# michaelnny/muzero

Measured on AMD Instinct MI355X. Metric: self-play MCTS sims/sec (env-steps/sec = value / sims_per_move), higher is better.
Workload: dtype f32

## Files before the change

muzero_amd/csrc/mz_search_fast.h:

```cpp
#pragma once
#include <type_traits>

#include "mz_search.h"

namespace mz {

#ifndef MZ_FAST_RD
#define MZ_FAST_RD 3
#endif
#ifndef MZ_FAST_RD256
#define MZ_FAST_RD256 4
#endif
#ifndef MZ_FAST_RD_GEN
#define MZ_FAST_RD_GEN 2
#endif
constexpr int fast_rd(int planes, int ac) { return planes == 256 ? MZ_FAST_RD256 : (ac == 2 ? MZ_FAST_RD : MZ_FAST_RD_GEN); }
#ifndef MZ_FAST_HW
#define MZ_FAST_HW 1
#endif
constexpr bool kFastHW = MZ_FAST_HW != 0;
#ifndef MZ_FAST_SC
#define MZ_FAST_SC 1
#endif
#ifndef MZ_FAST_AX
#define MZ_FAST_AX 1
#endif
constexpr bool kFastSC = MZ_FAST_SC != 0, kFastAX = MZ_FAST_AX != 0;

struct FastWeights {
    const float4* stream;
    unsigned bytes;
    const float* wact;
};

typedef unsigned int u32x4 __attribute__((ext_vector_type(4)));

struct WSrc {
    __amdgpu_buffer_rsrc_t r;
    int base;
    int cur;
};

__device__ __forceinline__ WSrc make_wsrc(const void* p, unsigned bytes, int base) {
    WSrc w;
    w.r = __builtin_amdgcn_make_buffer_rsrc(const_cast<void*>(p), 0, (int)bytes, 0x00020000);
    w.base = base;
    w.cur = base;
    return w;
}

__device__ __forceinline__ float4 bload(const WSrc& w, int voff, int block) {
    const u32x4 v = __builtin_amdgcn_raw_buffer_load_b128(w.r, voff, w.base + block * 1024, 0);
    return make_float4(__uint_as_float(v.x), __uint_as_float(v.y), __uint_as_float(v.z), __uint_as_float(v.w));
}

__device__ __forceinline__ float comp(const float4& v, int i) { return i == 0 ? v.x : (i == 1 ? v.y : (i == 2 ? v.z : v.w)); }

template <int P, int TR, int TV, int RD, int XG_ = 5>
struct FastCfg {
    static constexpr int NT = P / 64;
    static constexpr int XG = XG_;
    static constexpr int I_D1 = 0, I_D2 = I_D1 + XG, I_R1 = I_D2 + 4, I_R2 = I_R1 + 4, I_V1 = I_R2 + TR, I_V2 = I_V1 + 4, I_END = I_V2 + TV;
    static constexpr int SL = (I_END + RD - 1) / RD * RD;
};

template <typename C, int RD, int I>
__device__ __forceinline__ void prefetch_slot(float4 (&ring)[RD][C::NT], WSrc& ws, int voff) {
    constexpr int T = (I + RD - 1) % C::SL;
#ifdef MZ_EXP_NOLOAD
    return;
#endif
    if constexpr (T < C::I_END) {
        int so = ws.cur;
        asm volatile("" : "+s"(so));
        ws.cur = so + (T + 1 == C::I_END ? -(C::I_END - 1) : 1) * C::NT * 1024;
#pragma unroll
        for (int j = 0; j < C::NT; j++) {
            const u32x4 v = __builtin_amdgcn_raw_buffer_load_b128(ws.r, voff + (j & 3) * 1024, so + (j >> 2) * 4096, 0);
            ring[T % RD][j] = make_float4(__uint_as_float(v.x), __uint_as_float(v.y), __uint_as_float(v.z), __uint_as_float(v.w));
        }
    }
}

template <int NT, bool LDS_READ, int NV = 0>
__device__ __forceinline__ void slot_schedule() {
    if (LDS_READ) __builtin_amdgcn_sched_group_barrier(0x100, 1, 0);
#pragma unroll
    for (int i = 0; i < NT; i++) {
        __builtin_amdgcn_sched_group_barrier(0x020, 1, 0);
        if (NV == 0) {
            __builtin_amdgcn_sched_group_barrier(0x008, 4, 0);
        } else {
#pragma unroll
            for (int m = 0; m < 2; m++) {
                __builtin_amdgcn_sched_group_barrier(0x008, 2, 0);
                __builtin_amdgcn_sched_group_barrier(0x002, NV, 0);
            }
        }
    }
    if (NV == 0) __builtin_amdgcn_sched_barrier(0);
    else __builtin_amdgcn_sched_barrier(0);
}

struct NoHook {
    template <int K>
    __device__ __forceinline__ void stage() {}
};

template <typename C, int RD, int I0, int G, int KG, bool FROM_LDS, int NV = 0, typename Hook = NoHook, int HK0 = 0>
struct WideSlots {
    static __device__ __forceinline__ void run(float4 (&ring)[RD][C::NT], WSrc& ws, int voff, const float4 (&xs)[5], const f32x4 (&hin)[4],
                                               int last_steps, f32x4 (&acc)[C::NT], Hook& hook) {
        constexpr int NT = C::NT, I = I0 + G;
        prefetch_slot<C, RD, I>(ring, ws, voff);
        hook.template stage<HK0 + G>();
        float b[4];
        if (FROM_LDS) {
            const float4 x = xs[G];
            b[0] = x.x; b[1] = x.y; b[2] = x.z; b[3] = x.w;
        } else {
            b[0] = hin[G][0]; b[1] = hin[G][1]; b[2] = hin[G][2]; b[3] = hin[G][3];
        }
        const float4(&w)[NT] = ring[I % RD];
#pragma unroll
        for (int j = 0; j < NT; j++) acc[j] = __builtin_amdgcn_mfma_f32_16x16x4f32(w[j].x, b[0], acc[j], 0, 0, 0);
        if (G + 1 < KG || last_steps > 1) {
#pragma unroll
            for (int j = 0; j < NT; j++) acc[j] = __builtin_amdgcn_mfma_f32_16x16x4f32(w[j].y, b[1], acc[j], 0, 0, 0);
        }
        if (G + 1 < KG || last_steps > 2) {
#pragma unroll
            for (int j = 0; j < NT; j++) acc[j] = __builtin_amdgcn_mfma_f32_16x16x4f32(w[j].z, b[2], acc[j], 0, 0, 0);
        }
        if (G + 1 < KG || last_steps > 3) {
#pragma unroll
            for (int j = 0; j < NT; j++) acc[j] = __builtin_amdgcn_mfma_f32_16x16x4f32(w[j].w, b[3], acc[j], 0, 0, 0);
        }
        slot_schedule<NT, false, NV>();
        if constexpr (G + 1 < KG) WideSlots<C, RD, I0, G + 1, KG, FROM_LDS, NV, Hook, HK0>::run(ring, ws, voff, xs, hin, last_steps, acc, hook);
    }
};

template <typename C, int RD, int I0, int D, int TO, int NV = 0, typename Hook = NoHook, int HK0 = 0>
struct SplitSlots {
    static __device__ __forceinline__ void run(float4 (&ring)[RD][C::NT], WSrc& ws, int voff, const f32x4 (&hin)[C::NT], f32x4 (&acc)[TO],
                                               Hook& hook) {
        constexpr int NT = C::NT, I = I0 + D, KPS = NT / TO;
        static_assert(NT % TO == 0, "tiles per slot");
        prefetch_slot<C, RD, I>(ring, ws, voff);
        hook.template stage<HK0 + D>();
        const float4(&w)[NT] = ring[I % RD];
#pragma unroll
        for (int kk = 0; kk < KPS; kk++) {
            const int kb = D * KPS + kk;
#pragma unroll
            for (int st = 0; st < 4; st++) {
#pragma unroll
                for (int t = 0; t < TO; t++)
                    acc[t] = __builtin_amdgcn_mfma_f32_16x16x4f32(comp(w[kk * TO + t], st), hin[kb][st], acc[t], 0, 0, 0);
            }
        }
        slot_schedule<NT, false, NV>();
        if constexpr (D + 1 < TO) SplitSlots<C, RD, I0, D + 1, TO, NV, Hook, HK0>::run(ring, ws, voff, hin, acc, hook);
    }
};

template <typename C, int RD, int I>
struct PadSlots {
    static __device__ __forceinline__ void run(float4 (&ring)[RD][C::NT], WSrc& ws, int voff) {
        if constexpr (I < C::SL) {
            prefetch_slot<C, RD, I>(ring, ws, voff);
            __builtin_amdgcn_sched_barrier(0);
            PadSlots<C, RD, I + 1>::run(ring, ws, voff);
        }
    }
};

__device__ __forceinline__ float opaque_f32(unsigned int bits) {
    asm("" : "+s"(bits));
    return __uint_as_float(bits);
}
__device__ __forceinline__ float fmin2(float a, float b) { return __builtin_amdgcn_fmed3f(a, b, opaque_f32(0xff800000u)); }
__device__ __forceinline__ float fmax2(float a, float b) { return __builtin_amdgcn_fmed3f(a, b, opaque_f32(0x7f800000u)); }
typedef unsigned int u32x2 __attribute__((ext_vector_type(2)));
__device__ __forceinline__ float rows_min(float v) {
    u32x2 r = __builtin_amdgcn_permlane16_swap(__float_as_uint(v), __float_as_uint(v), false, false);
    v = fmin2(__uint_as_float(r[0]), __uint_as_float(r[1]));
    r = __builtin_amdgcn_permlane32_swap(__float_as_uint(v), __float_as_uint(v), false, false);
    return fmin2(__uint_as_float(r[0]), __uint_as_float(r[1]));
}
__device__ __forceinline__ float rows_max(float v) {
    u32x2 r = __builtin_amdgcn_permlane16_swap(__float_as_uint(v), __float_as_uint(v), false, false);
    v = fmax2(__uint_as_float(r[0]), __uint_as_float(r[1]));
    r = __builtin_amdgcn_permlane32_swap(__float_as_uint(v), __float_as_uint(v), false, false);
    return fmax2(__uint_as_float(r[0]), __uint_as_float(r[1]));
}

template <int N>
__device__ __forceinline__ void relu_tiles(f32x4 (&a)[N]) {
    const float inf = opaque_f32(0x7f800000u);
#pragma unroll
    for (int j = 0; j < N; j++) {
#pragma unroll
        for (int r = 0; r < 4; r++) a[j][r] = __builtin_amdgcn_fmed3f(a[j][r], 0.0f, inf);
    }
}

template <int TO>
__device__ __forceinline__ float head_logit(const float* PB, int n, int e) {
    const int t = n >> 4, idx = ((t * 64 + ((n & 15) >> 2) * 16 + e) << 2) + (n & 3);
    const float c0 = PB[idx], c1 = PB[idx + TO * 256], c2 = PB[idx + 2 * TO * 256], c3 = PB[idx + 3 * TO * 256];
    return ((c0 + c1) + c2) + c3;
}

template <int NT>
__device__ __forceinline__ void root_inference_fast(const MlpNet& net, const MlpLds& o, float* lds, float4* scr, float* hid0, float* pi0, int tid, int wave,
                                                    int lane, bool active) {
    const int q = lane >> 4;
    const float* bias = lds;
    MZ_ROOT_TS_START();
    f32x4 h1[NT];
    if (active) {
        const MlpLayer& L0 = net.L[L_REP0];
        const float4* wp = reinterpret_cast<const float4*>(L0.w) + (size_t)(NT * wave) * L0.kg * 64 + lane;
#pragma unroll
        for (int j = 0; j < NT; j++) {
            const float4 bv = *reinterpret_cast<const float4*>(bias + L0.b_lds + (NT * wave + j) * 16 + q * 4);
            h1[j] = f32x4{bv.x, bv.y, bv.z, bv.w};
        }
        float4 w0[NT], w1[NT];
#pragma unroll
        for (int j = 0; j < NT; j++) w0[j] = ldg4(&wp[(size_t)j * L0.kg * 64]);
        for (int g = 0; g < L0.kg; g += 2) {
            const int g1 = g + 1 < L0.kg ? g + 1 : g, g2 = g + 2 < L0.kg ? g + 2 : g;
#pragma unroll
            for (int j = 0; j < NT; j++) w1[j] = ldg4(&wp[((size_t)j * L0.kg + g1) * 64]);
            mma_block<NT>(h1, w0, reinterpret_cast<const float4*>(lds + o.X)[g * 64 + lane], g + 1 < L0.kg ? 4 : L0.last_steps);
#pragma unroll
            for (int j = 0; j < NT; j++) w0[j] = ldg4(&wp[((size_t)j * L0.kg + g2) * 64]);
            if (g + 1 < L0.kg) mma_block<NT>(h1, w1, reinterpret_cast<const float4*>(lds + o.X)[(g + 1) * 64 + lane], g + 2 < L0.kg ? 4 : L0.last_steps);
        }
        relu_tiles<NT>(h1);
        MZ_ROOT_TS(0);
        const MlpLayer& L1 = net.L[L_REP1];
        const float4* wq = reinterpret_cast<const float4*>(L1.w) + lane;
        f32x4 acc2[4];
#pragma unroll
        for (int t = 0; t < 4; t++) {
            const float4 bv = *reinterpret_cast<const float4*>(bias + L1.b_lds + t * 16 + q * 4);
            acc2[t] = wave == 0 ? f32x4{bv.x, bv.y, bv.z, bv.w} : f32x4{0.0f, 0.0f, 0.0f, 0.0f};
        }
        float4 wa[4], wb[4];
#pragma unroll
        for (int t = 0; t < 4; t++) wa[t] = ldg4(&wq[((size_t)t * L1.kg + NT * wave) * 64]);
#pragma unroll
        for (int kk = 0; kk < NT; kk += 2) {
#pragma unroll
            for (int t = 0; t < 4; t++) wb[t] = ldg4(&wq[((size_t)t * L1.kg + NT * wave + (kk + 1 < NT ? kk + 1 : kk)) * 64]);
#pragma unroll
            for (int st = 0; st < 4; st++) {
#pragma unroll
                for (int t = 0; t < 4; t++) acc2[t] = __builtin_amdgcn_mfma_f32_16x16x4f32(comp(wa[t], st), h1[kk][st], acc2[t], 0, 0, 0);
            }
#pragma unroll
            for (int t = 0; t < 4; t++) wa[t] = ldg4(&wq[((size_t)t * L1.kg + NT * wave + (kk + 2 < NT ? kk + 2 : kk)) * 64]);
            if (kk + 1 < NT) {
#pragma unroll
                for (int st = 0; st < 4; st++) {
#pragma unroll
                    for (int t = 0; t < 4; t++) acc2[t] = __builtin_amdgcn_mfma_f32_16x16x4f32(comp(wb[t], st), h1[kk + 1][st], acc2[t], 0, 0, 0);
                }
            }
        }
#pragma unroll
        for (int t = 0; t < 4; t++) scr[(wave * 4 + t) * 64 + lane] = make_float4(acc2[t][0], acc2[t][1], acc2[t][2], acc2[t][3]);
    }
    __syncthreads();
    MZ_ROOT_TS(1);
    if (active) {
        auto tile = [&](int t) {
            const float4 c0 = scr[(0 * 4 + t) * 64 + lane], c1 = scr[(1 * 4 + t) * 64 + lane], c2 = scr[(2 * 4 + t) * 64 + lane], c3 = scr[(3 * 4 + t) * 64 + lane];
            return f32x4{((c0.x + c1.x) + c2.x) + c3.x, ((c0.y + c1.y) + c2.y) + c3.y, ((c0.z + c1.z) + c2.z) + c3.z, ((c0.w + c1.w) + c2.w) + c3.w};
        };
        const f32x4 h0 = tile(0), h1_ = tile(1), h2 = tile(2), h3 = tile(3);
        float mn = h0[0], mx = h0[0];
#pragma unroll
        for (int r = 0; r < 4; r++) { mn = fmin2(h0[r], mn); mx = fmax2(h0[r], mx); }
#pragma unroll
        for (int r = 0; r < 4; r++) { mn = fmin2(h1_[r], mn); mx = fmax2(h1_[r], mx); }
#pragma unroll
        for (int r = 0; r < 4; r++) { mn = fmin2(h2[r], mn); mx = fmax2(h2[r], mx); }
#pragma unroll
        for (int r = 0; r < 4; r++) { mn = fmin2(h3[r], mn); mx = fmax2(h3[r], mx); }
        mn = rows_min(mn);
        mx = rows_max(mx);
        const float d = (mx - mn) + 1e-8f;
        f32x4 hw = h0;
        if (wave == 1) hw = h1_;
        if (wave == 2) hw = h2;
        if (wave == 3) hw = h3;
        const float4 hs = make_float4((hw[0] - mn) / d, (hw[1] - mn) / d, (hw[2] - mn) / d, (hw[3] - mn) / d);
        reinterpret_cast<float4*>(lds + o.HS)[wave * 64 + lane] = hs;
        if (hid0) *reinterpret_cast<float4*>(hid0 + wave * 16 + q * 4) = hs;
    }
    __syncthreads();
    MZ_ROOT_TS(2);
    if (active) {
        const MlpLayer& L2 = net.L[L_POL0];
        const float4* wp = reinterpret_cast<const float4*>(L2.w) + (size_t)(NT * wave) * L2.kg * 64 + lane;
        f32x4 p1[NT];
#pragma unroll
        for (int j = 0; j < NT; j++) {
            const float4 bv = *reinterpret_cast<const float4*>(bias + L2.b_lds + (NT * wave + j) * 16 + q * 4);
            p1[j] = f32x4{bv.x, bv.y, bv.z, bv.w};
        }
        float4 w0[NT], w1[NT];
#pragma unroll
        for (int j = 0; j < NT; j++) w0[j] = ldg4(&wp[(size_t)j * L2.kg * 64]);
#pragma unroll
        for (int g = 0; g < 4; g += 2) {
#pragma unroll
            for (int j = 0; j < NT; j++) w1[j] = ldg4(&wp[((size_t)j * L2.kg + g + 1) * 64]);
            mma_block_full<NT>(p1, w0, reinterpret_cast<const float4*>(lds + o.HS)[g * 64 + lane]);
#pragma unroll
            for (int j = 0; j < NT; j++) w0[j] = ldg4(&wp[((size_t)j * L2.kg + (g + 2 < 4 ? g + 2 : g)) * 64]);
            mma_block_full<NT>(p1, w1, reinterpret_cast<const float4*>(lds + o.HS)[(g + 1) * 64 + lane]);
        }
        relu_tiles<NT>(p1);
        MZ_ROOT_TS(3);
        const MlpLayer& L3 = net.L[L_POL1];
        const float4* wq = reinterpret_cast<const float4*>(L3.w) + (size_t)(NT * wave) * 64 + lane;
        const float4 bv = *reinterpret_cast<const float4*>(bias + L3.b_lds + q * 4);
        f32x4 accp = wave == 0 ? f32x4{bv.x, bv.y, bv.z, bv.w} : f32x4{0.0f, 0.0f, 0.0f, 0.0f};
        float4 wv[NT];
#pragma unroll
        for (int kk = 0; kk < NT; kk++) wv[kk] = ldg4(&wq[kk * 64]);
#pragma unroll
        for (int kk = 0; kk < NT; kk++) {
#pragma unroll
            for (int st = 0; st < 4; st++) accp = __builtin_amdgcn_mfma_f32_16x16x4f32(comp(wv[kk], st), p1[kk][st], accp, 0, 0, 0);
        }
        scr[wave * 64 + lane] = make_float4(accp[0], accp[1], accp[2], accp[3]);
    }
    __syncthreads();
    MZ_ROOT_TS(4);
    if (active && wave == 0) {
        const float4 c0 = scr[lane], c1 = scr[64 + lane], c2 = scr[128 + lane], c3 = scr[192 + lane];
        float* pl = lds + o.LG + (lane & 15) * o.lg_stride + q * 4;
        pl[0] = ((c0.x + c1.x) + c2.x) + c3.x; pl[1] = ((c0.y + c1.y) + c2.y) + c3.y;
        pl[2] = ((c0.z + c1.z) + c2.z) + c3.z; pl[3] = ((c0.w + c1.w) + c2.w) + c3.w;
    }
    __syncthreads();
    if (active) row_softmax(lds + o.LG + (tid >> 4) * o.lg_stride, pi0 + (tid >> 4) * net.A, net.A, tid & 15);
    __syncthreads();
    MZ_ROOT_TS(5);
}

template <int P, int TR, int TV, bool FUSE = false, int AC = 0, bool HW = false, bool SPB = false>
__global__ __launch_bounds__(HW ? 2 * WG_THREADS : WG_THREADS) __attribute__((amdgpu_waves_per_eu(HW ? 2 : 1, HW ? 2 : 1))) void k_search_fast(const SearchParams Pm, const FastWeights FW) {
    constexpr bool TWO = AC == 2;
    constexpr int RD = fast_rd(P, AC);
    constexpr bool SC = AC == 10 && kFastSC, AX = AC == 10 && kFastAX;
    using C = FastCfg<P, SC ? 0 : TR, SC ? 0 : TV, RD, AX ? 4 : 5>;
    constexpr int NT = C::NT;
    extern __shared__ __attribute__((aligned(16))) unsigned char smem[];
    float* lds = reinterpret_cast<float*>(smem);
    const int wave8 = __builtin_amdgcn_readfirstlane((int)threadIdx.x >> 6);
    const bool main_w = !HW || wave8 < WG_WAVES;
    const int tid = threadIdx.x & (WG_THREADS - 1), e = tid >> 4, a0 = tid & 15, lane = tid & 63;
    const int wave = wave8 & (WG_WAVES - 1);
    const int env_g = blockIdx.x * TILE_E + e;
    const bool env_ok = env_g < Pm.B;
    if constexpr (FUSE) { if (main_w) fused_env_pre(Pm, a0, env_g, env_ok); }
    const bool hwx = HW && (Pm.hwx & 1) != 0;
    const bool hwx2 = HW && (Pm.hwx & 2) != 0;
    const MlpNet& net = Pm.net;
    const int root_layers[4] = {L_REP0, L_REP1, L_POL0, L_POL1};
    const float warm = main_w ? prefetch_root_weights(net, root_layers, 4, tid) : 0.0f;
    const MlpLds& o = Pm.o;
    float* pi0 = reinterpret_cast<float*>(smem + Pm.t_pi0);
    const float** src = reinterpret_cast<const float**>(smem + Pm.t_ptr);
    float** dst = reinterpret_cast<float**>(smem + Pm.t_ptr) + 16;

    MZ_STAMP_DECL
    MZ_STAMP_START();
    if (main_w) {
        stage_biases(net, lds, tid);
        if (!HW) tree2_init(smem, Pm, tid, env_ok, env_g);
        if (a0 == 0) {
            src[e] = env_ok ? Pm.obs + (size_t)env_g * net.in_dim : nullptr;
            dst[e] = env_ok ? Pm.hidden + (size_t)env_g * Pm.NN * net.H : nullptr;
        }
    }
    __syncthreads();
    MZ_STAMP(2);
    if (!HW) root_noise_lanes(smem, Pm, e, a0, env_g, env_ok);
    if (main_w) load_obs(net, lds + o.X, src, tid);
    __syncthreads();
    MZ_STAMP(15);
    if (HW && !main_w) {
        tree2_init(smem, Pm, tid, env_ok, env_g);
        root_noise_lanes(smem, Pm, e, a0, env_g, env_ok);
    }
    {
        const int e2r = lane & 15, env2r = blockIdx.x * TILE_E + e2r;
        float* hid0 = (main_w && env2r < Pm.B) ? Pm.hidden + (size_t)env2r * Pm.NN * 64 : nullptr;
        root_inference_fast<NT>(net, o, lds, reinterpret_cast<float4*>(lds + o.H1), hid0, pi0, tid, wave, lane, main_w);
    }
    if (Pm.S < 0) Pm.hidden[0] = warm;
    __syncthreads();
    {
        MZ_ROOT_TS_START();
        SearchParams Pr = Pm;
        if constexpr (AC == 10 || AC == 4) Pr.A = AC;
        if constexpr (TWO) Pr.A = 2;
        if constexpr (SPB) { Pr.noise_mode = 2; Pr.has_mask = 1; }
        if (main_w && env_ok) root_prior_group(smem, Pr, e, a0, env_g);
        MZ_ROOT_TS(6);
    }

    const int voff = lane * 16;
    WSrc ws = make_wsrc(FW.stream, FW.bytes, wave * C::SL * NT * 1024);
    ws.cur = ws.base + (RD - 1) * NT * 1024;
    float4 ring[RD][NT];
    if (main_w) {
#pragma unroll
        for (int i = 0; i < RD - 1; i++) {
#pragma unroll
            for (int j = 0; j < NT; j++) ring[i][j] = bload(ws, voff, i * NT + j);
        }
    }
    const int x_last = AX ? 4 : (TWO ? 1 : net.L[L_DYN0].last_steps);
    const int e2 = lane & 15, q = lane >> 4;
    const int env2 = blockIdx.x * TILE_E + e2;
    const bool env2_ok = env2 < Pm.B;
    const unsigned hid_sel = (unsigned)((env_ok ? env_g : 0) * Pm.NN * 64 + a0 * 4) * 4u;
    const unsigned hid_mma = (unsigned)((env2_ok ? env2 : 0) * Pm.NN * 64 + wave * 16 + q * 4) * 4u;
    char* const hid_base = reinterpret_cast<char*>(Pm.hidden);
    const float* bias = lds;
    float4 w_sr[NT], w_sv[NT];
    if constexpr (SC) {
        if (main_w) {
            const float4* wr = reinterpret_cast<const float4*>(net.L[L_REW1].w);
            const float4* wv = reinterpret_cast<const float4*>(net.L[L_VAL1].w);
#pragma unroll
            for (int j = 0; j < NT; j++) {
                w_sr[j] = ldg4(&wr[(NT * wave + j) * 64 + q * 16]);
                w_sv[j] = ldg4(&wv[(NT * wave + j) * 64 + q * 16]);
            }
        }
    }
    auto scalar_head = [&](const f32x4 (&x)[NT], const float4 (&w)[NT], float b0, float* part ) {
        float pacc = (wave == 0 && q == 0) ? b0 : 0.0f;
#pragma unroll
        for (int j = 0; j < NT; j++) {
            pacc = fmaf(x[j][0], w[j].x, pacc); pacc = fmaf(x[j][1], w[j].y, pacc);
            pacc = fmaf(x[j][2], w[j].z, pacc); pacc = fmaf(x[j][3], w[j].w, pacc);
        }
        u32x2 r = __builtin_amdgcn_permlane16_swap(__float_as_uint(pacc), __float_as_uint(pacc), false, false);
        pacc = __uint_as_float(r[0]) + __uint_as_float(r[1]);
        r = __builtin_amdgcn_permlane32_swap(__float_as_uint(pacc), __float_as_uint(pacc), false, false);
        pacc = __uint_as_float(r[0]) + __uint_as_float(r[1]);
        if (q == 0) part[wave * 256 + e2 * 4] = pacc;
    };
    float4* const PB = reinterpret_cast<float4*>(lds + o.H1);
    float4* const PBr = reinterpret_cast<float4*>(lds + o.V1);
    float4* const PBv = PBr + 4 * TR * 64;
    float* const rew_x = lds + o.OUT;
    const float4 zero4 = make_float4(0.f, 0.f, 0.f, 0.f);
    const float4 xs0[5] = {zero4, zero4, zero4, zero4, zero4};
    NoHook nohook;
    float* const zeros = lds + o.PM;
    if (main_w && tid < 128) zeros[tid] = 0.0f;
    const float* const b_d2 = wave == 0 ? bias + net.L[L_DYN1].b_lds : zeros;
    const float* const b_r2 = wave == 0 ? bias + net.L[L_REW1].b_lds : zeros;
    const float* const b_v2 = wave == 0 ? bias + net.L[L_VAL1].b_lds : zeros;
    __syncthreads();
    MZ_STAMP(0);

    int resume = 0;
    const int cp0 = env_ok ? Pm.cur[env_g] : 0, op0 = env_ok ? Pm.opp[env_g] : 0;
    SearchParams Pl = Pm;
    if constexpr (AC == 10 || AC == 4) Pl.A = AC;
    if constexpr (TWO) Pl.A = 2;
    if constexpr (SPB) { Pl.board = 1; Pl.has_bounds = 1; Pl.noise_mode = 2; Pl.rng_mode = 1; Pl.discount = 1.0; }
    Tree2Env T;
    tree2_env_init(T, Pl);
    auto normalise_store = [&](const f32x4 h0, const f32x4 h1_, const f32x4 h2, const f32x4 h3, int s) {
        float mn = h0[0], mx = h0[0];
#pragma unroll
        for (int r = 0; r < 4; r++) {
            mn = fmin2(h0[r], mn); mx = fmax2(h0[r], mx);
        }
#pragma unroll
        for (int r = 0; r < 4; r++) {
            mn = fmin2(h1_[r], mn); mx = fmax2(h1_[r], mx);
        }
#pragma unroll
        for (int r = 0; r < 4; r++) {
            mn = fmin2(h2[r], mn); mx = fmax2(h2[r], mx);
        }
#pragma unroll
        for (int r = 0; r < 4; r++) {
            mn = fmin2(h3[r], mn); mx = fmax2(h3[r], mx);
        }
        mn = rows_min(mn);
        mx = rows_max(mx);
        const float d = (mx - mn) + 1e-8f;
        f32x4 hw = h0;
        if (wave == 1) hw = h1_;
        if (wave == 2) hw = h2;
        if (wave == 3) hw = h3;
        const float4 hs = make_float4((hw[0] - mn) / d, (hw[1] - mn) / d, (hw[2] - mn) / d, (hw[3] - mn) / d);
        reinterpret_cast<float4*>(lds + o.HS)[wave * 64 + lane] = hs;
        if (env2_ok) *reinterpret_cast<float4*>(hid_base + (size_t)(hid_mma + (unsigned)(s + 1) * 256u)) = hs;
    };
    constexpr bool MSE = AC == 10;
    float4* const HT = reinterpret_cast<float4*>(lds + o.HN);
    auto reduce_tile = [&]() {
        const float4 c0 = PB[(0 * 4 + wave) * 64 + lane], c1 = PB[(1 * 4 + wave) * 64 + lane], c2 = PB[(2 * 4 + wave) * 64 + lane],
                     c3 = PB[(3 * 4 + wave) * 64 + lane];
        HT[wave * 64 + lane] = make_float4(((c0.x + c1.x) + c2.x) + c3.x, ((c0.y + c1.y) + c2.y) + c3.y, ((c0.z + c1.z) + c2.z) + c3.z,
                                           ((c0.w + c1.w) + c2.w) + c3.w);
    };
    auto read_h = [&](f32x4 (&h)[4]) {
#pragma unroll
        for (int t = 0; t < 4; t++) {
            const float4 v = HT[t * 64 + lane];
            h[t] = f32x4{v.x, v.y, v.z, v.w};
        }
    };
    const bool cat_heads = !MSE && (TWO || AC == 4 || (net.Sr != 1 && net.Sv != 1));
    if (HW && !main_w) {
        for (int s = 0; s < Pm.S; s++) {
            __syncthreads();
            __syncthreads();
            __syncthreads();
            if (hwx) {
                f32x4 h[4];
                read_h(h);
                normalise_store(h[0], h[1], h[2], h[3], s);
            }
            __syncthreads();
            if (hwx2 && cat_heads) {
                const float* fr = reinterpret_cast<const float*>(PBr);
                const bool r0 = a0 < net.Sr, r1 = a0 + 16 < net.Sr;
                const float lr0 = head_logit<TR>(fr, r0 ? a0 : 0, e), lr1 = head_logit<TR>(fr, r1 ? a0 + 16 : 0, e);
                const float rew = row2_logits_to_scalar(lr0, lr1, r0, r1, net.Sr, a0);
                if (a0 == 0) rew_x[e] = rew;
            }
            __syncthreads();
        }
        return;
    }
    for (int s = 0; s < Pm.S; s++) {
        tree2_select<false, TWO ? 2 : 0>(smem, Pl, tid, env_ok, env_g, T, cp0, op0, resume);
        const int lp = T.lp, la = T.la;
        {
            float* X = lds + o.X;
            float4 hv = make_float4(0.f, 0.f, 0.f, 0.f);
            if (env_ok) hv = *reinterpret_cast<const float4*>(hid_base + (size_t)(hid_sel + (unsigned)lp * 256u));
            reinterpret_cast<float4*>(X)[(a0 >> 2) * 64 + (a0 & 3) * 16 + e] = hv;
            if constexpr (AX) { if (a0 == 0) reinterpret_cast<int*>(smem + Pm.t_sel)[e * 4 + 1] = env_ok ? la : 0; }
            else X[pk_act(a0, e, 4)] = (a0 == la && a0 < Pm.A) ? 1.0f : 0.0f;
        }
        __syncthreads();
        MZ_STAMP(1);
        f32x4 h1[NT], h[4];
        {
            const float* b1 = bias + net.L[L_DYN0].b_lds + wave * NT * 16;
#pragma unroll
            for (int j = 0; j < NT; j++) {
                const float4 bv = *reinterpret_cast<const float4*>(b1 + j * 16 + q * 4);
                h1[j] = f32x4{bv.x, bv.y, bv.z, bv.w};
            }
            float4 xs[5];
#pragma unroll
            for (int g = 0; g < C::XG; g++) xs[g] = reinterpret_cast<const float4*>(lds + o.X)[g * 64 + lane];
            float4 wa4[NT];
            if constexpr (AX) {
                const int la2 = reinterpret_cast<const int*>(smem + Pm.t_sel)[e2 * 4 + 1];
                const float4* wc = reinterpret_cast<const float4*>(FW.wact + la2 * P + wave * NT * 16 + q * 4);
#pragma unroll
                for (int j = 0; j < NT; j++) wa4[j] = wc[j * 4];
            }
            WideSlots<C, RD, C::I_D1, 0, C::XG, true>::run(ring, ws, voff, xs, h, x_last, h1, nohook);
            if constexpr (AX) {
#pragma unroll
                for (int j = 0; j < NT; j++) { h1[j][0] += wa4[j].x; h1[j][1] += wa4[j].y; h1[j][2] += wa4[j].z; h1[j][3] += wa4[j].w; }
            }
            relu_tiles<NT>(h1);
            MZ_STAMP(3);
            f32x4 acc2[4];
#pragma unroll
            for (int t = 0; t < 4; t++) {
                const float4 bv = *reinterpret_cast<const float4*>(b_d2 + t * 16 + q * 4);
                acc2[t] = f32x4{bv.x, bv.y, bv.z, bv.w};
            }
            SplitSlots<C, RD, C::I_D2, 0, 4>::run(ring, ws, voff, h1, acc2, nohook);
#pragma unroll
            for (int t = 0; t < 4; t++) PB[(wave * 4 + t) * 64 + lane] = make_float4(acc2[t][0], acc2[t][1], acc2[t][2], acc2[t][3]);
        }
        __syncthreads();
        MZ_STAMP(4);
        reduce_tile();
        __syncthreads();
        read_h(h);
        if (!hwx) normalise_store(h[0], h[1], h[2], h[3], s);
        MZ_STAMP(5);
        {
            f32x4 r1[NT];
            const float* b1 = bias + net.L[L_REW0].b_lds + wave * NT * 16;
#pragma unroll
            for (int j = 0; j < NT; j++) {
                const float4 bv = *reinterpret_cast<const float4*>(b1 + j * 16 + q * 4);
                r1[j] = f32x4{bv.x, bv.y, bv.z, bv.w};
            }
            WideSlots<C, RD, C::I_R1, 0, 4, false>::run(ring, ws, voff, xs0, h, 4, r1, nohook);
            relu_tiles<NT>(r1);
            if constexpr (SC) {
                scalar_head(r1, w_sr, bias[net.L[L_REW1].b_lds], reinterpret_cast<float*>(PBr));
            } else {
            f32x4 accr[TR];
#pragma unroll
            for (int t = 0; t < TR; t++) {
                const float4 bv = *reinterpret_cast<const float4*>(b_r2 + t * 16 + q * 4);
                accr[t] = f32x4{bv.x, bv.y, bv.z, bv.w};
            }
            SplitSlots<C, RD, C::I_R2, 0, TR>::run(ring, ws, voff, r1, accr, nohook);
#pragma unroll
            for (int t = 0; t < TR; t++) PBr[(wave * TR + t) * 64 + lane] = make_float4(accr[t][0], accr[t][1], accr[t][2], accr[t][3]);
            }
        }
        __syncthreads();
        MZ_STAMP(6);
        {
            f32x4 v1[NT];
            const float* b1 = bias + net.L[L_VAL0].b_lds + wave * NT * 16;
#pragma unroll
            for (int j = 0; j < NT; j++) {
                const float4 bv = *reinterpret_cast<const float4*>(b1 + j * 16 + q * 4);
                v1[j] = f32x4{bv.x, bv.y, bv.z, bv.w};
            }
            float4 xs[5];
#pragma unroll
            for (int g = 0; g < 4; g++) xs[g] = reinterpret_cast<const float4*>(lds + o.HS)[g * 64 + lane];
            xs[4] = zero4;
            WideSlots<C, RD, C::I_V1, 0, 4, true>::run(ring, ws, voff, xs, h, 4, v1, nohook);
            relu_tiles<NT>(v1);
            if constexpr (SC) {
                scalar_head(v1, w_sv, bias[net.L[L_VAL1].b_lds], reinterpret_cast<float*>(PBv));
            } else {
            f32x4 accv[TV];
#pragma unroll
            for (int t = 0; t < TV; t++) {
                const float4 bv = *reinterpret_cast<const float4*>(b_v2 + t * 16 + q * 4);
                accv[t] = f32x4{bv.x, bv.y, bv.z, bv.w};
            }
            SplitSlots<C, RD, C::I_V2, 0, TV>::run(ring, ws, voff, v1, accv, nohook);
#pragma unroll
            for (int t = 0; t < TV; t++) PBv[(wave * TV + t) * 64 + lane] = make_float4(accv[t][0], accv[t][1], accv[t][2], accv[t][3]);
            }
            PadSlots<C, RD, C::I_END>::run(ring, ws, voff);
        }
        Backup2Pre bpre;
        if constexpr (TWO) bpre = tree2_backup_prefetch<2>(smem, Pl, tid, env_ok, s, T);
        __syncthreads();
        MZ_STAMP(7);
        {
            const float* fr = reinterpret_cast<const float*>(PBr);
            const float* fv = reinterpret_cast<const float*>(PBv);
            float rew, val;
            if constexpr (MSE) {
                rew = head_logit<TR>(fr, 0, e);
                val = head_logit<TV>(fv, 0, e);
            } else
            if (hwx2 && cat_heads) {
                const bool v0 = a0 < net.Sv, v1 = a0 + 16 < net.Sv;
                const float lv0 = head_logit<TV>(fv, v0 ? a0 : 0, e), lv1 = head_logit<TV>(fv, v1 ? a0 + 16 : 0, e);
                rew = rew_x[e];
                val = row2_logits_to_scalar(lv0, lv1, v0, v1, net.Sv, a0);
            } else if (cat_heads) {
                const bool hr0 = a0 < net.Sr, hr1 = a0 + 16 < net.Sr, hv0 = a0 < net.Sv, hv1 = a0 + 16 < net.Sv;
                const float l0[2] = {head_logit<TR>(fr, hr0 ? a0 : 0, e), head_logit<TV>(fv, hv0 ? a0 : 0, e)};
                const float l1[2] = {head_logit<TR>(fr, hr1 ? a0 + 16 : 0, e), head_logit<TV>(fv, hv1 ? a0 + 16 : 0, e)};
                const bool h0[2] = {hr0, hv0}, h1[2] = {hr1, hv1};
                const int SS[2] = {net.Sr, net.Sv};
                float out[2];
                rows2_logits_to_scalars(l0, l1, h0, h1, SS, a0, out);
                rew = out[0];
                val = out[1];
            } else {
            if (net.Sr == 1) {
                rew = head_logit<TR>(fr, 0, e);
            } else {
                const bool r0 = a0 < net.Sr, r1 = a0 + 16 < net.Sr;
                const float lr0 = head_logit<TR>(fr, r0 ? a0 : 0, e), lr1 = head_logit<TR>(fr, r1 ? a0 + 16 : 0, e);
                rew = row2_logits_to_scalar(lr0, lr1, r0, r1, net.Sr, a0);
            }
            if (net.Sv == 1) {
                val = head_logit<TV>(fv, 0, e);
            } else {
                const bool v0 = a0 < net.Sv, v1 = a0 + 16 < net.Sv;
                const float lv0 = head_logit<TV>(fv, v0 ? a0 : 0, e), lv1 = head_logit<TV>(fv, v1 ? a0 + 16 : 0, e);
                val = row2_logits_to_scalar(lv0, lv1, v0, v1, net.Sv, a0);
            }
            }
            MZ_STAMP(8);
            resume = tree2_backup<TWO ? 2 : 0, (AC > 2 ? AC : 0), TWO>(smem, Pl, tid, env_ok, s, rew, val, T, &bpre);
        }
        MZ_STAMP(9);
    }
    typedef const __attribute__((address_space(4))) SearchParams* late_params_t;
    late_params_t late = (late_params_t)__builtin_amdgcn_kernarg_segment_ptr();
    asm volatile("" : "+s"(late));
    const SearchParams& Pt = *(const SearchParams*)late;
    bool stepped = false;
    if constexpr (FUSE && TWO) {
        if (Pt.fenv.env.kind == ENV_CARTPOLE) {
            CartPolePre pre;
            const bool stepper = env_ok && a0 == 0;
            if (stepper) cartpole_prefetch(Pt.fenv, env_g, pre);
            int action = 0;
            double rootv = 0.0;
            if (env_ok) {
                SearchParams Pf = Pt;
                Pf.A = 2;
                tree2_finish_group(smem, Pf, e, a0, env_g, action, rootv);
            }
            if (stepper) cartpole_step_prefetched(Pt.fenv, env_g, pre, action, rootv, reinterpret_cast<const double*>(smem + Pt.t_tmp) + e * 2);
            stepped = true;
        }
    }
    if constexpr (FUSE && AC == 10) {
        if (Pt.fenv.env.kind == ENV_TICTACTOE && Pt.fenv.env.nn <= 16 && Pt.A <= 16) {
            BoardSmallPre pre;
            if (env_ok) board_small_prefetch(Pt.fenv, env_g, a0, pre);
            int action = 0;
            double rootv = 0.0;
            if (env_ok) {
                SearchParams Pf = Pt;
                Pf.A = 10;
                if constexpr (SPB) { Pf.deterministic = 0; Pf.has_mask = 1; Pf.rng_mode = 1; }
                tree2_finish_group(smem, Pf, e, a0, env_g, action, rootv);
                board_step_small_prefetched(Pt.fenv, env_g, a0, pre, action, rootv, reinterpret_cast<const double*>(smem + Pt.t_tmp) + e * 10);
            }
            stepped = true;
        }
    }
    if (!stepped) {
        if (env_ok) tree2_finish_group(smem, Pt, e, a0, env_g);
        if constexpr (FUSE)
            if (env_ok) env_step_group(Pt.fenv, env_g, a0);
    }
    MZ_STAMP(10);
    MZ_STAMP_FLUSH(Pm);
}

}
```

Measured before the change: 293.6 million.

## Stream root-inference weights through a unified buffer-load ring across all four layers

Replaces the per-layer double-buffered global loads in root inference with a single kRootRD-deep ring of buffer-resource loads that runs continuously across rep0, rep1, pol0 and pol1. The first entries are primed at kernel start, before the bias staging and observation load, so the weight fetch latency is hidden behind setup work. The root noise computation moves into the side lambda that the helper waves execute during the pol0 phase. The search-loop weight ring priming is moved ahead of root_prior_group. This uses more registers for the window and adds template complexity. It also assumes NT is divisible by 4.

```diff
diff --git a/muzero_amd/csrc/mz_search_fast.h b/muzero_amd/csrc/mz_search_fast.h
--- a/muzero_amd/csrc/mz_search_fast.h
+++ b/muzero_amd/csrc/mz_search_fast.h
@@ -213,65 +213,174 @@
     return ((c0 + c1) + c2) + c3;
 }
 
+#ifndef MZ_ROOT_RD
+#define MZ_ROOT_RD 3
+#endif
+constexpr int kRootRD = MZ_ROOT_RD;
+static_assert(kRootRD >= 2, "the root's window needs an entry in flight");
+
+struct RootSrc {
+    __amdgpu_buffer_rsrc_t r0, r1, r2, r3;
+    int kg0;
+    int pad;
+    int b0;
+    int ts0;
+    int wq;
+};
+
 template <int NT>
+__device__ __forceinline__ RootSrc make_root_src(const MlpNet& net, int wave) {
+    auto rsrc = [](const MlpLayer& L) {
+        return __builtin_amdgcn_make_buffer_rsrc(const_cast<float*>(L.w), 0, L.n_tiles * L.kg * 1024, 0x00020000);
+    };
+    RootSrc rs;
+    rs.r0 = rsrc(net.L[L_REP0]); rs.r1 = rsrc(net.L[L_REP1]); rs.r2 = rsrc(net.L[L_POL0]); rs.r3 = rsrc(net.L[L_POL1]);
+    rs.kg0 = net.L[L_REP0].kg;
+    rs.pad = (int)((unsigned)(kRootRD - (int)((unsigned)rs.kg0 % kRootRD)) % kRootRD);
+    rs.ts0 = rs.kg0 * 1024;
+    rs.b0 = NT * wave * rs.ts0;
+    rs.wq = NT * wave * 1024;
+    return rs;
+}
+
+__device__ __forceinline__ float4 rload(__amdgpu_buffer_rsrc_t r, int voff, int soff) {
+    const u32x4 v = __builtin_amdgcn_raw_buffer_load_b128(r, voff, soff, 0);
+    return make_float4(__uint_as_float(v.x), __uint_as_float(v.y), __uint_as_float(v.z), __uint_as_float(v.w));
+}
+
+template <int NT>
+__device__ __forceinline__ void root_req_rep0(float4 (&w)[NT], const RootSrc& rs, int voff, int g) {
+    int so = rs.b0 + g * 1024;
+    asm volatile("" : "+s"(so));
+#pragma unroll
+    for (int j = 0; j < NT; j++) {
+        w[j] = rload(rs.r0, voff, so);
+        so += rs.ts0;
+    }
+}
+
+template <int NT, int N>
+__device__ __forceinline__ void root_req_fixed(float4 (&w)[NT], const RootSrc& rs, int voff) {
+    static_assert(NT % 4 == 0, "a rep1 slot holds whole input blocks");
+    if constexpr (N < 4) {
+        constexpr int KPS = NT / 4;
+        int so = rs.wq;
+        asm volatile("" : "+s"(so));
+#pragma unroll
+        for (int kl = 0; kl < KPS; kl++) {
+#pragma unroll
+            for (int t = 0; t < 4; t++) {
+                const int kk = N * KPS + kl;
+                w[kl * 4 + t] = rload(rs.r1, voff + (kk & 3) * 1024, so + (t * 4 * NT + (kk & ~3)) * 1024);
+            }
+        }
+    } else if constexpr (N < 8) {
+        int so = rs.wq * 4;
+        asm volatile("" : "+s"(so));
+#pragma unroll
+        for (int j = 0; j < NT; j++) w[j] = rload(rs.r2, voff + (N - 4) * 1024, so + j * 4096);
+    } else if constexpr (N == 8) {
+        int so = rs.wq;
+        asm volatile("" : "+s"(so));
+#pragma unroll
+        for (int kk = 0; kk < NT; kk++) w[kk] = rload(rs.r3, voff + (kk & 3) * 1024, so + (kk >> 2) * 4096);
+    }
+}
+
+template <int NT, int N>
+__device__ __forceinline__ void root_prime_fixed(float4 (&win)[kRootRD][NT], const RootSrc& rs, int voff) {
+    if constexpr (N < kRootRD - 1) {
+        if (rs.kg0 + N < kRootRD - 1) root_req_fixed<NT, N>(win[N % kRootRD], rs, voff);
+        root_prime_fixed<NT, N + 1>(win, rs, voff);
+    }
+}
+template <int NT>
+__device__ __forceinline__ void root_prime(float4 (&win)[kRootRD][NT], const RootSrc& rs, int voff) {
+#pragma unroll
+    for (int en = 0; en < kRootRD; en++) {
+        const int g = (int)((unsigned)(en + rs.kg0) % kRootRD);
+        if (g < kRootRD - 1 && g < rs.kg0) root_req_rep0<NT>(win[en], rs, voff, g);
+    }
+    root_prime_fixed<NT, 0>(win, rs, voff);
+}
+
+template <int NT, bool LAST, int I>
+__device__ __forceinline__ void root_rep0_slots(float4 (&win)[kRootRD][NT], const RootSrc& rs, int voff, const float4* X4, int v, int last_steps,
+                                                f32x4 (&h1)[NT]) {
+    if constexpr (I < kRootRD) {
+        const int g = v + I - rs.pad;
+        if (g >= 0) {
+            if constexpr (!LAST || I == 0) root_req_rep0<NT>(win[(I + kRootRD - 1) % kRootRD], rs, voff, g + kRootRD - 1);
+            else root_req_fixed<NT, I - 1>(win[(I - 1) % kRootRD], rs, voff);
+            const float4 x = X4[g * 64];
+            if constexpr (LAST && I == kRootRD - 1) mma_block<NT>(h1, win[I], x, last_steps);
+            else mma_block_full<NT>(h1, win[I], x);
+            slot_schedule<NT, true>();
+        }
+        root_rep0_slots<NT, LAST, I + 1>(win, rs, voff, X4, v, last_steps, h1);
+    }
+}
+
+template <int NT, int D>
+__device__ __forceinline__ void root_rep1_slots(float4 (&win)[kRootRD][NT], const RootSrc& rs, int voff, const f32x4 (&h1)[NT], f32x4 (&acc2)[4]) {
+    if constexpr (D < 4) {
+        constexpr int KPS = NT / 4;
+        root_req_fixed<NT, D + kRootRD - 1>(win[(D + kRootRD - 1) % kRootRD], rs, voff);
+        const float4(&w)[NT] = win[D % kRootRD];
+#pragma unroll
+        for (int kl = 0; kl < KPS; kl++) {
+#pragma unroll
+            for (int st = 0; st < 4; st++) {
+#pragma unroll
+                for (int t = 0; t < 4; t++)
+                    acc2[t] = __builtin_amdgcn_mfma_f32_16x16x4f32(comp(w[kl * 4 + t], st), h1[D * KPS + kl][st], acc2[t], 0, 0, 0);
+            }
+        }
+        slot_schedule<NT, false>();
+        root_rep1_slots<NT, D + 1>(win, rs, voff, h1, acc2);
+    }
+}
+
+template <int NT, int G>
+__device__ __forceinline__ void root_pol0_slots(float4 (&win)[kRootRD][NT], const RootSrc& rs, int voff, const float4* HS4, f32x4 (&p1)[NT]) {
+    if constexpr (G < 4) {
+        root_req_fixed<NT, 4 + G + kRootRD - 1>(win[(4 + G + kRootRD - 1) % kRootRD], rs, voff);
+        const float4 x = HS4[G * 64];
+        mma_block_full<NT>(p1, win[(4 + G) % kRootRD], x);
+        slot_schedule<NT, true>();
+        root_pol0_slots<NT, G + 1>(win, rs, voff, HS4, p1);
+    }
+}
+
+template <int NT, typename Side>
 __device__ __forceinline__ void root_inference_fast(const MlpNet& net, const MlpLds& o, float* lds, float4* scr, float* hid0, float* pi0, int tid, int wave,
-                                                    int lane, bool active) {
-    const int q = lane >> 4;
+                                                    int lane, bool active, float4 (&win)[kRootRD][NT], const RootSrc& rs, Side& side) {
+    const int q = lane >> 4, voff = lane * 16;
     const float* bias = lds;
     MZ_ROOT_TS_START();
     f32x4 h1[NT];
     if (active) {
         const MlpLayer& L0 = net.L[L_REP0];
-        const float4* wp = reinterpret_cast<const float4*>(L0.w) + (size_t)(NT * wave) * L0.kg * 64 + lane;
 #pragma unroll
         for (int j = 0; j < NT; j++) {
             const float4 bv = *reinterpret_cast<const float4*>(bias + L0.b_lds + (NT * wave + j) * 16 + q * 4);
             h1[j] = f32x4{bv.x, bv.y, bv.z, bv.w};
         }
-        float4 w0[NT], w1[NT];
-#pragma unroll
-        for (int j = 0; j < NT; j++) w0[j] = ldg4(&wp[(size_t)j * L0.kg * 64]);
-        for (int g = 0; g < L0.kg; g += 2) {
-            const int g1 = g + 1 < L0.kg ? g + 1 : g, g2 = g + 2 < L0.kg ? g + 2 : g;
-#pragma unroll
-            for (int j = 0; j < NT; j++) w1[j] = ldg4(&wp[((size_t)j * L0.kg + g1) * 64]);
-            mma_block<NT>(h1, w0, reinterpret_cast<const float4*>(lds + o.X)[g * 64 + lane], g + 1 < L0.kg ? 4 : L0.last_steps);
-#pragma unroll
-            for (int j = 0; j < NT; j++) w0[j] = ldg4(&wp[((size_t)j * L0.kg + g2) * 64]);
-            if (g + 1 < L0.kg) mma_block<NT>(h1, w1, reinterpret_cast<const float4*>(lds + o.X)[(g + 1) * 64 + lane], g + 2 < L0.kg ? 4 : L0.last_steps);
-        }
+        const float4* X4 = reinterpret_cast<const float4*>(lds + o.X) + lane;
+        const int v_last = rs.kg0 + rs.pad - kRootRD;
+        int v = 0;
+        for (; v < v_last; v += kRootRD) root_rep0_slots<NT, false, 0>(win, rs, voff, X4, v, 4, h1);
+        root_rep0_slots<NT, true, 0>(win, rs, voff, X4, v, L0.last_steps, h1);
         relu_tiles<NT>(h1);
         MZ_ROOT_TS(0);
         const MlpLayer& L1 = net.L[L_REP1];
-        const float4* wq = reinterpret_cast<const float4*>(L1.w) + lane;
         f32x4 acc2[4];
 #pragma unroll
         for (int t = 0; t < 4; t++) {
             const float4 bv = *reinterpret_cast<const float4*>(bias + L1.b_lds + t * 16 + q * 4);
             acc2[t] = wave == 0 ? f32x4{bv.x, bv.y, bv.z, bv.w} : f32x4{0.0f, 0.0f, 0.0f, 0.0f};
         }
-        float4 wa[4], wb[4];
-#pragma unroll
-        for (int t = 0; t < 4; t++) wa[t] = ldg4(&wq[((size_t)t * L1.kg + NT * wave) * 64]);
-#pragma unroll
-        for (int kk = 0; kk < NT; kk += 2) {
-#pragma unroll
-            for (int t = 0; t < 4; t++) wb[t] = ldg4(&wq[((size_t)t * L1.kg + NT * wave + (kk + 1 < NT ? kk + 1 : kk)) * 64]);
-#pragma unroll
-            for (int st = 0; st < 4; st++) {
-#pragma unroll
-                for (int t = 0; t < 4; t++) acc2[t] = __builtin_amdgcn_mfma_f32_16x16x4f32(comp(wa[t], st), h1[kk][st], acc2[t], 0, 0, 0);
-            }
-#pragma unroll
-            for (int t = 0; t < 4; t++) wa[t] = ldg4(&wq[((size_t)t * L1.kg + NT * wave + (kk + 2 < NT ? kk + 2 : kk)) * 64]);
-            if (kk + 1 < NT) {
-#pragma unroll
-                for (int st = 0; st < 4; st++) {
-#pragma unroll
-                    for (int t = 0; t < 4; t++) acc2[t] = __builtin_amdgcn_mfma_f32_16x16x4f32(comp(wb[t], st), h1[kk + 1][st], acc2[t], 0, 0, 0);
-                }
-            }
-        }
+        root_rep1_slots<NT, 0>(win, rs, voff, h1, acc2);
 #pragma unroll
         for (int t = 0; t < 4; t++) scr[(wave * 4 + t) * 64 + lane] = make_float4(acc2[t][0], acc2[t][1], acc2[t][2], acc2[t][3]);
     }
@@ -305,36 +414,22 @@
     }
     __syncthreads();
     MZ_ROOT_TS(2);
+    if (!active) side();
     if (active) {
         const MlpLayer& L2 = net.L[L_POL0];
-        const float4* wp = reinterpret_cast<const float4*>(L2.w) + (size_t)(NT * wave) * L2.kg * 64 + lane;
         f32x4 p1[NT];
 #pragma unroll
         for (int j = 0; j < NT; j++) {
             const float4 bv = *reinterpret_cast<const float4*>(bias + L2.b_lds + (NT * wave + j) * 16 + q * 4);
             p1[j] = f32x4{bv.x, bv.y, bv.z, bv.w};
         }
-        float4 w0[NT], w1[NT];
-#pragma unroll
-        for (int j = 0; j < NT; j++) w0[j] = ldg4(&wp[(size_t)j * L2.kg * 64]);
-#pragma unroll
-        for (int g = 0; g < 4; g += 2) {
-#pragma unroll
-            for (int j = 0; j < NT; j++) w1[j] = ldg4(&wp[((size_t)j * L2.kg + g + 1) * 64]);
-            mma_block_full<NT>(p1, w0, reinterpret_cast<const float4*>(lds + o.HS)[g * 64 + lane]);
-#pragma unroll
-            for (int j = 0; j < NT; j++) w0[j] = ldg4(&wp[((size_t)j * L2.kg + (g + 2 < 4 ? g + 2 : g)) * 64]);
-            mma_block_full<NT>(p1, w1, reinterpret_cast<const float4*>(lds + o.HS)[(g + 1) * 64 + lane]);
-        }
+        root_pol0_slots<NT, 0>(win, rs, voff, reinterpret_cast<const float4*>(lds + o.HS) + lane, p1);
         relu_tiles<NT>(p1);
         MZ_ROOT_TS(3);
         const MlpLayer& L3 = net.L[L_POL1];
-        const float4* wq = reinterpret_cast<const float4*>(L3.w) + (size_t)(NT * wave) * 64 + lane;
         const float4 bv = *reinterpret_cast<const float4*>(bias + L3.b_lds + q * 4);
         f32x4 accp = wave == 0 ? f32x4{bv.x, bv.y, bv.z, bv.w} : f32x4{0.0f, 0.0f, 0.0f, 0.0f};
-        float4 wv[NT];
-#pragma unroll
-        for (int kk = 0; kk < NT; kk++) wv[kk] = ldg4(&wq[kk * 64]);
+        const float4(&wv)[NT] = win[8 % kRootRD];
 #pragma unroll
         for (int kk = 0; kk < NT; kk++) {
 #pragma unroll
@@ -376,6 +471,10 @@
     const bool hwx2 = HW && (Pm.hwx & 2) != 0;
     const MlpNet& net = Pm.net;
     const int root_layers[4] = {L_REP0, L_REP1, L_POL0, L_POL1};
+    const int voff = lane * 16;
+    const RootSrc rs = make_root_src<NT>(net, wave);
+    float4 rwin[kRootRD][NT];
+    if (main_w) root_prime<NT>(rwin, rs, voff);
     const float warm = main_w ? prefetch_root_weights(net, root_layers, 4, tid) : 0.0f;
     const MlpLds& o = Pm.o;
     float* pi0 = reinterpret_cast<float*>(smem + Pm.t_pi0);
@@ -398,17 +497,27 @@
     if (main_w) load_obs(net, lds + o.X, src, tid);
     __syncthreads();
     MZ_STAMP(15);
-    if (HW && !main_w) {
-        tree2_init(smem, Pm, tid, env_ok, env_g);
-        root_noise_lanes(smem, Pm, e, a0, env_g, env_ok);
-    }
+    if (HW && !main_w) tree2_init(smem, Pm, tid, env_ok, env_g);
+    auto root_side = [&]() {
+        if (HW) root_noise_lanes(smem, Pm, e, a0, env_g, env_ok);
+    };
     {
         const int e2r = lane & 15, env2r = blockIdx.x * TILE_E + e2r;
         float* hid0 = (main_w && env2r < Pm.B) ? Pm.hidden + (size_t)env2r * Pm.NN * 64 : nullptr;
-        root_inference_fast<NT>(net, o, lds, reinterpret_cast<float4*>(lds + o.H1), hid0, pi0, tid, wave, lane, main_w);
+        root_inference_fast<NT>(net, o, lds, reinterpret_cast<float4*>(lds + o.H1), hid0, pi0, tid, wave, lane, main_w, rwin, rs, root_side);
     }
     if (Pm.S < 0) Pm.hidden[0] = warm;
     __syncthreads();
+    WSrc ws = make_wsrc(FW.stream, FW.bytes, wave * C::SL * NT * 1024);
+    ws.cur = ws.base + (RD - 1) * NT * 1024;
+    float4 ring[RD][NT];
+    if (main_w) {
+#pragma unroll
+        for (int i = 0; i < RD - 1; i++) {
+#pragma unroll
+            for (int j = 0; j < NT; j++) ring[i][j] = bload(ws, voff, i * NT + j);
+        }
+    }
     {
         MZ_ROOT_TS_START();
         SearchParams Pr = Pm;
@@ -419,17 +528,6 @@
         MZ_ROOT_TS(6);
     }
 
-    const int voff = lane * 16;
-    WSrc ws = make_wsrc(FW.stream, FW.bytes, wave * C::SL * NT * 1024);
-    ws.cur = ws.base + (RD - 1) * NT * 1024;
-    float4 ring[RD][NT];
-    if (main_w) {
-#pragma unroll
-        for (int i = 0; i < RD - 1; i++) {
-#pragma unroll
-            for (int j = 0; j < NT; j++) ring[i][j] = bload(ws, voff, i * NT + j);
-        }
-    }
     const int x_last = AX ? 4 : (TWO ? 1 : net.L[L_DYN0].last_steps);
     const int e2 = lane & 15, q = lane >> 4;
     const int env2 = blockIdx.x * TILE_E + e2;
```

New measurement: 293.6 million (median of 3 runs). No clear change (+0.0%).
